# tenstack/batch-scheduler

Measured on AMD Instinct MI355X. Metric: pod x node fit evals/sec, higher is better.
Workload: dtype int64; 1 GPU; cfg3/tail: 10000 pods / 2000 groups / 5000 nodes, 5 int64 lanes (cpu, mem, eph, pods, gpu), seed 20260921; stages=prefilter+filter+tally+ready, parallelism=single GPU

## Files before the change

### batch-scheduler_amd/csrc/bs_fast.hpp

```cpp
#pragma once

#include "bs_kernels.hpp"
#include "bs_filter_t.hpp"

#ifdef BS_NT_TABLES
#define BS_TBL_STORE(p, v) __builtin_nontemporal_store((v), (p))
#else
#define BS_TBL_STORE(p, v) (*(p) = (v))
#endif
namespace bs {

template <bool INL = false>
__device__ __forceinline__ void arm_tally(const GroupsDev& gr, const BatchDev& b, const BatchParams& prm, uint32_t i, uint32_t nthreads);

__device__ __forceinline__ const uint8_t* range_glocal(const BatchDev& b) { return reinterpret_cast<const uint8_t*>(b.pod_ranges); }
__device__ __forceinline__ const uint32_t* range_start(const BatchDev& b, uint32_t G) { return b.pod_ranges + (G + 3u) / 4u; }
__device__ __forceinline__ const uint32_t* range_lfirst(const BatchDev& b, uint32_t G, uint32_t pod_blocks) { return range_start(b, G) + pod_blocks + 1u; }
__device__ __forceinline__ bool range_local_on(const BatchDev& b, const BatchParams& prm) {
  return b.pod_ranges && prm.do_tally && prm.do_ready && !prm.filter_deny;
}

#if BS_EMIT_MAIN
__global__ void k_pods_prep(unsigned long long* tables, uint32_t ntab, uint32_t* gstat, uint32_t ngstat, uint32_t* kcount, uint32_t* gcount, uint32_t G) {
  const uint32_t t = blockIdx.x * blockDim.x + threadIdx.x, nt = gridDim.x * blockDim.x;
  for (uint32_t i = t; i < ntab; i += nt) tables[i] = 0ull;
  for (uint32_t i = t; i < G; i += nt) gcount[i] = 0;
  for (uint32_t i = t; i < ngstat; i += nt) gstat[i] = BS_INF;
  if (t == 0 && kcount) *kcount = 0;
}
#endif

#if BS_EMIT_MAIN
__global__ void k_pod_pairs(PodsDev pods, uint32_t G, const uint32_t* rep, const uint32_t* id, uint32_t* pclass, unsigned long long* slots, uint32_t mask,
                            uint32_t hash_keep, uint32_t* gstat, uint32_t* ppair, unsigned long long* pair_next, const uint32_t* kcount, int32_t tag,
                            int32_t* hinfo, uint32_t* gcount) {
  const uint32_t i = blockIdx.x * blockDim.x + threadIdx.x;
  if (i == 0 && hinfo) {
    __hip_atomic_store(reinterpret_cast<unsigned long long*>(&hinfo[4]), ((unsigned long long)(uint32_t)tag << 32) | *kcount, __ATOMIC_RELAXED, __HIP_MEMORY_SCOPE_SYSTEM);
  }
  {
    const int32_t gq = i < pods.p ? pods.group[i] : -1;
    const bool in = gq >= 0 && (uint32_t)gq < G;
    wave_aggregated_add(gcount, in ? (uint32_t)gq : 0u, in);
  }
  if (i >= pods.p) return;
  const uint32_t c = id[rep[i]];
  if (pclass) pclass[i] = c;
  const int32_t gi = pods.group[i];
  if (gi < 0 || (uint32_t)gi >= G) { ppair[i] = BS_INF; return; }
  atomicMin(&gstat[gi], i);
  if (!(pods.flags[i] & BS_POD_LAST_PERMITTED)) {
    atomicMin(&gstat[(size_t)G + gi], i);
    if (pods.owner[i] != 0) atomicMin(&gstat[(size_t)2 * G + gi], i);
  }
  const uint64_t h = mix64(((uint64_t)(uint32_t)gi << 32) | c);
  bool winner;
// ... 447 lines not shown
      b.nodew[nodew_pair(stride, s, w) + 1] = ~holds;
    }
    if (blk == 0 && threadIdx.x == 0) {
#pragma unroll
      for (int j = 0; j < 4; ++j) b.nodew[nodew_ref_lane(stride, s, j)] = (uint64_t)ms.v[j];
      b.nodew[nodew_ref_flags(stride, s)] = ff;
    }
  }
}

template <int TS>
__global__ __launch_bounds__(kTblChunk) void k_fast_query_tables(PodsDev pods, GroupsDev gr, NodesDev nd, BatchDev b, BatchDev bt, BatchParams prm,
                                                                 const TableDesc* forced, uint32_t nchunks, uint32_t query_blocks) {
  BS_STAMP(1, 0);
  if (blockIdx.x < query_blocks) fast_query_thread<TS>(pods, gr, b, prm, blockIdx.x * kTblChunk + threadIdx.x, query_blocks * kTblChunk);
  else if (blockIdx.x < query_blocks + nchunks) tables_local_fast<TS>(nd, bt, prm, forced, blockIdx.x - query_blocks);
  else node_words_block<TS>(gr, nd, b, prm, blockIdx.x - query_blocks - nchunks);
  BS_STAMP(1, 7);
}

template <int NL>
__device__ __forceinline__ unsigned long long rows_cover(unsigned long long m, const int64_t (&a)[BS_MAX_LANES], const int64_t (&r)[BS_MAX_LANES]) {
  asm volatile("s_mov_b64 exec, %[m]\n\tv_cmpx_ge_i64 vcc, %[a0], %[r0]\n\tv_cmpx_ge_i64 vcc, %[a1], %[r1]\n\tv_cmpx_ge_i64 vcc, %[a2], %[r2]\n\t"
               "v_cmpx_ge_i64 vcc, %[a3], %[r3]\n\ts_mov_b64 %[m], exec\n\ts_mov_b64 exec, -1"
               : [m] "+s"(m)
               : [a0] "v"(a[0]), [r0] "v"(r[0]), [a1] "v"(a[1]), [r1] "v"(r[1]), [a2] "v"(a[2]), [r2] "v"(r[2]), [a3] "v"(a[3]), [r3] "v"(r[3])
               : "vcc");
#pragma unroll
  for (int j = 4; j < NL; ++j)
    asm volatile("s_mov_b64 exec, %[m]\n\tv_cmpx_ge_i64 vcc, %[a], %[r]\n\ts_mov_b64 %[m], exec\n\ts_mov_b64 exec, -1" : [m] "+s"(m) : [a] "v"(a[j]), [r] "v"(r[j]) : "vcc");
  return m;
}
#ifndef BS_SCAN_BALLOT
#define BS_SCAN_BALLOT 1
#endif
constexpr uint32_t kSpinBound = 1u << 18;
__device__ __forceinline__ void test_chaos_delay() {
#ifdef BS_TEST_CHAOS
  uint32_t h = (blockIdx.x + 1u) * 2654435761u ^ (uint32_t)wall_clock64() * 40503u;
  h ^= h >> 15; h *= 2246822519u; h ^= h >> 13;
  for (uint32_t s = 0; s < (h & 15u); ++s) __builtin_amdgcn_s_sleep(127);
#endif
}
constexpr uint32_t kStepSlotsMax = 256;
__device__ __forceinline__ bool step_wait(const uint32_t* word, uint32_t base, uint32_t need, int32_t* h_err) {
  uint32_t spins = 0;
  while ((uint32_t)(ld_agent(word) - base) < need) {
    __builtin_amdgcn_s_sleep(1);
    if (++spins > kSpinBound) { if (h_err) __hip_atomic_store(h_err, 1, __ATOMIC_RELAXED, __HIP_MEMORY_SCOPE_SYSTEM); return false; }
  }
  return true;
}
constexpr uint32_t kScanRecChunks = 64;
constexpr uint32_t kFeasRecGroups = 32;
#ifndef BS_GATHER_DIRECT
#define BS_GATHER_DIRECT 8
#endif
constexpr uint32_t kGatherDirectBlocks = BS_GATHER_DIRECT;
constexpr uint32_t kRecStride = 32;
constexpr uint32_t kTkSlots = 32, kTkTab = 48, kTkP1 = 64, kTkDone = 64 + 16 * 16, kTkWays = 16, kTkWords = 64 + 2 * 16 * 16;
__device__ __forceinline__ void spread_add(uint32_t* words, uint32_t who) {
  (void)__hip_atomic_fetch_add(&words[16u * (who % kTkWays)], 1u, __ATOMIC_RELAXED, __HIP_MEMORY_SCOPE_AGENT);
}
__device__ __forceinline__ bool spread_wait(const uint32_t* words, uint32_t base, uint32_t need, int32_t* h_err) {
  uint32_t spins = 0;
  for (;;) {
    uint32_t v = lane_id() < (int)kTkWays ? ld_agent(&words[16u * (uint32_t)lane_id()]) : 0u;
#pragma unroll
    for (int o = 1; o < (int)kTkWays; o <<= 1) v += (uint32_t)__shfl_xor((int)v, o);
    v = (uint32_t)__builtin_amdgcn_readfirstlane((int)v);
    if ((uint32_t)(v - base) >= need) return true;
    __builtin_amdgcn_s_sleep(4);
    if (++spins > kSpinBound) { if (h_err && lane_id() == 0) __hip_atomic_store(h_err, 1, __ATOMIC_RELAXED, __HIP_MEMORY_SCOPE_SYSTEM); return false; }
  }
}
template <int TS, bool REGS = false>
__device__ __forceinline__ void table_scan_block(const NodesDev& nd, const BatchDev& b, const BatchParams& prm, const TableDesc* forced, uint32_t chunk, uint32_t nchunks,
                                                 uint32_t share, uint32_t nshares, uint32_t pod_blocks, uint32_t tk_pods0, uint32_t tk_tab0, const GroupsDev& gr,
                                                 const int64_t* ckeys, const uint32_t* cpres, uint32_t kcap, bool direct = false, uint32_t forced_cls = 0) {
  __shared__ unsigned long long s_wtot[BS_MAX_LANES][4];
  __shared__ uint32_t s_kp[BS_MAX_SCALARS];
  __shared__ unsigned long long s_off[BS_MAX_LANES];
  __shared__ uint32_t s_kpg[BS_MAX_SCALARS];
  __shared__ int64_t s_req[kStepSlotsMax][BS_MAX_LANES];
  __shared__ uint32_t s_qf[kStepSlotsMax];
  __shared__ uint32_t s_first[kStepSlotsMax];
  BS_STAMP(2, 0);
  const Shape<TS> sh(prm.S);
  const uint32_t L = sh.L(), S = sh.S(), LP = prm.LP;
  const uint32_t k = chunk * kTblChunk + threadIdx.x;
  const bool in_range = REGS ? k < nd.n : k < nd.m;
  const uint32_t n = REGS ? (in_range ? k : 0u) : (in_range ? nd.kmap[k] : 0u);
  const TableDesc d = REGS ? TableDesc{forced_cls, 0.7f} : *forced;
  const uint32_t fw = nd.fit[(size_t)d.cls * nd.fit_words + (n >> 5)];
  const uint8_t fl = nd.flags[n];
  const bool valid = in_range && (!REGS || !(fl & BS_NODE_SKIP_MASK));
  const uint32_t ap = nd.apres[n], rp = nd.rpres[n];
  int64_t al[BS_MAX_LANES], rq[BS_MAX_LANES];
#pragma unroll
  for (uint32_t j = 0; j < BS_MAX_LANES; ++j) {
    if (j < L) {
      al[j] = nd.alloc[(size_t)j * nd.stride + n];
      rq[j] = nd.req[(size_t)j * nd.stride + n];
    }
  }
  const uint32_t K = prm.k_host ? prm.k_host : *b.kclass;
  const uint32_t per = (K + nshares - 1u) / nshares, s_lo = share * per, s_hi = min(K, s_lo + per);
// ... 147 lines not shown
    uint32_t stp = 0, qf = 0x80000000u;
    int32_t tab = -1;
    unsigned long long rv[BS_MAX_LANES];
    if (!REGS && t < s_hi) {
      stp = ld_agent(&b.qstamp_s[t]);
      tab = (int32_t)ld_agent(reinterpret_cast<const uint32_t*>(&b.qtab_s[t]));
      qf = ld_agent(&b.qflags_s[t]);
#pragma unroll
      for (uint32_t j = 0; j < BS_MAX_LANES; ++j) rv[j] = j < L ? ld_agent64(&b.qreq_s[(size_t)t * LP + j]) : 0ull;
    }
    if (w == 0) {
#pragma unroll
      for (uint32_t j = 0; j < BS_MAX_LANES; ++j) {
        if (j < L) {
          const unsigned long long incl_c = wave_incl_scan_add_u64(cv[j]);
          const unsigned long long mine = bcast64(incl_c - cv[j], (int)(chunk & 63u));
          if (ch == 0) s_off[j] = mine;
        }
      }
#pragma unroll
      for (uint32_t s2 = 0; s2 < BS_MAX_SCALARS; ++s2) {
        if (s2 < S) {
          const uint32_t mn = wave_min_u32(ckp[s2]);
          if (ch == 0) s_kpg[s2] = mn;
        }
      }
    }
    if (!REGS && t < s_hi) {
      if (stp != prm.stamp || tab != 0) qf = 0x80000000u;
      s_qf[threadIdx.x] = qf;
#pragma unroll
      for (uint32_t j = 0; j < BS_MAX_LANES; ++j)
        if (j < L) s_req[threadIdx.x][j] = (int64_t)rv[j];
    }
  }
  __syncthreads();
  if constexpr (REGS) {
    if (!s_ok) return;
  }
  int64_t fin[BS_MAX_LANES];
  uint32_t keyrow = 0;
#pragma unroll
  for (uint32_t j = 0; j < BS_MAX_LANES; ++j) {
    fin[j] = 0;
    if (j < L) fin[j] = (int64_t)(incl[j] + s_off[j]);
  }
#pragma unroll
  for (uint32_t s2 = 0; s2 < BS_MAX_SCALARS; ++s2)
    if (s2 < S && k >= s_kpg[s2]) keyrow |= 1u << s2;
  BS_STAMP(2, 3);
  const uint32_t nmine = s_hi > s_lo ? s_hi - s_lo : 0u;
  const uint32_t smask = S ? ((1u << S) - 1u) : 0u;
  const uint32_t row0 = chunk * kTblChunk + ((uint32_t)w << 6);
  for (uint32_t t0 = 0; t0 < nmine; t0 += 4u) {
    uint32_t qf[4];
    int64_t r[4][BS_MAX_LANES];
#pragma unroll
    for (uint32_t u = 0; u < 4; ++u) {
      const uint32_t t = min(t0 + u, nmine - 1u);
      qf[u] = t0 + u < nmine ? s_qf[t] : 0x80000000u;
#pragma unroll
      for (uint32_t j = 0; j < BS_MAX_LANES; ++j) r[u][j] = j < L ? s_req[t][j] : 0;
    }
#pragma unroll
    for (uint32_t u = 0; u < 4; ++u) {
      const uint32_t nab = ~(qf[u] >> 16) & smask;
      unsigned long long m = (qf[u] & 0x80000000u) ? 0ull : __ballot(valid && (nab & ~keyrow) == 0u);
      static_assert(TS >= 0 && TS <= 4, "k_fast_step_a is instantiated for 0..4 scalar lanes (run_fast: step_a_possible)");
#if BS_SCAN_BALLOT
#pragma unroll
      for (uint32_t j = 0; j < 4u + (uint32_t)TS; ++j) m &= __ballot(fin[j] >= r[u][j]);
#else
      m = rows_cover<4 + TS>(m, fin, r[u]);
#endif
      if (m && lane_id() == 0) atomicMin(&s_first[t0 + u], row0 + (uint32_t)(__ffsll((long long)m) - 1));
    }
  }
  __syncthreads();
  BS_STAMP(2, 4);
  if constexpr (REGS) {
    if (direct) {
      for (uint32_t t = threadIdx.x; t < nmine; t += kTblChunk)
        st_pub<true>(&b.scan_rec[(size_t)chunk * kStepSlotsMax + s_lo + t], ((unsigned long long)prm.seq_inv << 32) | s_first[t]);
    } else {
      for (uint32_t t = threadIdx.x; t < nmine; t += kTblChunk)
        if (s_first[t] != BS_INF) atomicMin(&b.first_row64[s_lo + t], ((unsigned long long)prm.seq_inv << 32) | s_first[t]);
    }
    BS_STAMP(2, 7);
    return;
  }
  for (uint32_t t = threadIdx.x; t < nmine; t += kTblChunk) {
    if (s_first[t] == BS_INF) continue;
    atomicMin(&b.first_row[s_lo + t], s_first[t]);
  }
  BS_STAMP(2, 7);
}

__device__ __forceinline__ void step_filter_split(uint32_t K, uint32_t W, uint32_t target_waves, uint32_t& tiles, uint32_t& bpw, uint32_t& nchunk) {
  tiles = (2u * K + 63u) / 64u;
  uint32_t nsplit = max(1u, target_waves / max(tiles, 1u));
  nsplit = min(nsplit, max((W + 1u) / 2u, 1u));
  bpw = max(2u, (((W + nsplit - 1u) / nsplit + 1u) / 2u) * 2u);
  nchunk = (W + bpw - 1u) / bpw;
  if ((nchunk + 3u) / 4u > kFeasRecGroups) {
    bpw = ((W + 4u * kFeasRecGroups - 1u) / (4u * kFeasRecGroups) + 1u) / 2u * 2u;
    nchunk = (W + bpw - 1u) / bpw;
  }
}
template <int TS>
__device__ __forceinline__ void step_filter_block(const GroupsDev& gr, const NodesDev& nd, const BatchDev& b, const BatchParams& prm, const int64_t* ckeys,
                                                  const uint32_t* cpres, uint32_t kcap, uint32_t target_waves, uint32_t ustride, uint32_t bx, uint32_t nblocks,
                                                  bool direct, uint32_t tk_slots0, uint32_t slot_producers) {
  __shared__ uint32_t s_cnt[4][64];
  BS_STAMP_AT(4, 0, bx);
  const Shape<TS> sh(prm.S);
  const uint32_t gate = prm.eph_gate, K = prm.k_host ? prm.k_host : (uint32_t)__builtin_amdgcn_readfirstlane((int)*b.kclass), U = 2u * K;
  const uint32_t W = (nd.n + 63u) / 64u;
  if (!U || !W) return;
  uint32_t tiles, bpw, nchunk;
  step_filter_split(K, W, target_waves, tiles, bpw, nchunk);
  const uint32_t groups = (nchunk + 3u) / 4u;
  const int32_t leader0 = b.leader_epoch[0];
  LeaderPre lp0{}, lp1{};
  const bool two = prm.sop_leader0 >= 0 && prm.sop_leader0 != leader0;
  if (gr.g) {
    leader_pre_load(gr, leader0, sh, lp0);
    if (two) leader_pre_load(gr, prm.sop_leader0, sh, lp1); else lp1 = lp0;
  }
  bool waited = false;
  for (uint32_t bi = bx; bi < tiles * groups; bi += nblocks) {
    const uint32_t tile = bi % tiles, group = bi / tiles, chunk = group * 4u + (uint32_t)wave_id();
    const uint32_t src = tile * 64u + (uint32_t)lane_id();
    const bool second = src >= K;
    const uint32_t c = src < U ? (second ? src - K : src) : 0u;
    uint32_t cnt = 0;
    if (chunk < nchunk) {
      Res raw;
#pragma unroll
      for (uint32_t j = 0; j < BS_MAX_LANES; ++j)
        if (j < sh.L()) raw.v[j] = ckeys[(size_t)j * kcap + c];
      raw.present = cpres[c];
      Res cur;
      res_zero(cur, sh);
      res_add(cur, raw, sh, gate);
      LeaderPre lp = lp0;
      if (second) lp = lp1;
      const bool on = src < U && (second ? prm.sop_leader0 >= 0 : leader0 >= 0) && lp.have_mr;
      int64_t R[4], M[4];
      const uint32_t ff = filter_slot_values(cur, lp, sh, gate, R, M);
      filter_item<2, 4, true, true>(nd, b, U, ustride, tile, chunk * bpw, min(W, chunk * bpw + bpw), 0u,
                                    on ? (ff | ((uint32_t)BS_FL_EVALUATED << 8)) : ((uint32_t)BS_FL_NOT_RUN << 8), R, M, &cnt);
    }
    s_cnt[wave_id()][lane_id()] = cnt;
    BS_STAMP_AT(4, 1, bx);
    if (direct && b.h_rows) asm volatile("s_waitcnt vmcnt(0)" ::: "memory");
    __syncthreads();
    BS_STAMP_AT(4, 2, bx);
    if (wave_id() == 0 && src < U) {
      const uint32_t sum = s_cnt[0][lane_id()] + s_cnt[1][lane_id()] + s_cnt[2][lane_id()] + s_cnt[3][lane_id()];
      if (direct) {
        st_pub<true>(&b.feas_rec[(size_t)group * (2u * kStepSlotsMax) + src], ((unsigned long long)prm.seq_inv << 32) | sum);
      } else {
        if (!waited) { (void)step_wait(&b.ticket[kTkSlots], tk_slots0, slot_producers, b.h_err); waited = true; }
        if (sum) atomicAdd(&b.fu_feas[src], sum);
      }
    }
    __syncthreads();
  }
  BS_STAMP_AT(4, 7, bx);
}

template <int TS>
__device__ __forceinline__ void class_slots_block(const GroupsDev& gr, const BatchDev& b, const BatchParams& prm, const int64_t* ckeys, const uint32_t* cpres,
                                                  uint32_t kcap, uint32_t blk, bool zero_feas) {
  const Shape<TS> sh(prm.S);
#ifdef BS_TEST_OLD_ZERO
  zero_feas = true;
#endif
  const uint32_t gate = prm.eph_gate, K = prm.k_host ? prm.k_host : *b.kclass;
  const uint32_t c = blk * kTblChunk + threadIdx.x;
  Res raw;
  const uint32_t cc = c < K ? c : 0u;
#pragma unroll
  for (uint32_t j = 0; j < BS_MAX_LANES; ++j)
    if (j < sh.L()) raw.v[j] = ckeys[(size_t)j * kcap + cc];
  raw.present = cpres[cc];
  const int32_t leader0 = b.leader_epoch[0];
  const uint8_t panic0 = b.panic_epoch[0];
  LeaderPre lp0{}, lp1{};
  const bool two = prm.run_filter && prm.sop_leader0 >= 0 && prm.sop_leader0 != leader0;
  if (gr.g) {
    leader_pre_load(gr, leader0, sh, lp0);
    if (two) leader_pre_load(gr, prm.sop_leader0, sh, lp1); else lp1 = lp0;
  }
  if (c < K) {
    Res cur;
    res_zero(cur, sh);
    res_add(cur, raw, sh, gate);
    if (leader0 >= 0 && !panic0) {
      Res q;
      const uint32_t qfw = class_scan_query(cur, lp0, sh, gate, q);
      int64_t* dst = b.qreq_s + (size_t)c * prm.LP;
#pragma unroll
      for (uint32_t j = 0; j < BS_MAX_LANES; ++j)
        if (j < prm.LP) st_pub<true>(&dst[j], j < sh.L() ? q.v[j] : (int64_t)INT64_MIN);
      st_pub<true>(&b.qflags_s[c], qfw);
      st_pub<true>(&b.qtab_s[c], (int32_t)0);
      st_pub<true>(&b.first_row[c], BS_INF);
      st_pub<true>(&b.qstamp_s[c], prm.stamp);
    }
    if (prm.run_filter) {
// ... 126 lines not shown
    __syncthreads();
  }
  const uint32_t dx = bx * 256u + threadIdx.x;
  const uint32_t i = p0 == BS_INF ? dx : p0 + threadIdx.x;
  const bool valid = i < pods.p && (p0 == BS_INF || i < p1);
  uint8_t code0 = 0, st0 = 0;
  int32_t gi0 = BS_POD_NOT_GROUPED;
  uint32_t qpos0 = 0, pclass0 = 0, pair0 = BS_INF;
  uint32_t lfirst = BS_INF;
  if (valid) { code0 = b.tcode[i]; st0 = b.stage[i]; gi0 = pods.group[i]; qpos0 = b.qpos[i]; pclass0 = b.pclass[i]; pair0 = b.ppair[i]; }
  if (INL && valid && range_local_on(b, prm)) lfirst = range_lfirst(b, gr.g, query_blocks)[i];
  const uint32_t K = prm.k_host ? prm.k_host : *b.kclass;
  const int32_t leader_now = b.leader_epoch[0];
  if (threadIdx.x < 64) {
    uint32_t found = BS_INF;
    for (uint32_t b0 = 0; b0 < query_blocks && found == BS_INF; b0 += 64u) {
      const uint32_t bk = b0 + threadIdx.x;
      uint32_t v = BS_INF;
      if (bk < query_blocks) {
        const unsigned long long w = INL ? ld_agent64(&b.first_reach64[bk]) : b.first_reach64[bk];
        if ((uint32_t)(w >> 32) == prm.seq_inv) v = (uint32_t)w;
      }
      const unsigned long long any = __ballot(v != BS_INF);
      if (any) found = (uint32_t)__shfl((int)v, __ffsll((long long)any) - 1);
    }
    if (threadIdx.x == 0) s_first_reach = found;
  }
  const bool owned = valid && (st0 & ST_OWNED);
  const bool walk = owned && (st0 & ST_ELIG);
  const bool grouped = valid && gi0 >= 0 && (uint32_t)gi0 < gr.g;
  uint32_t row_q = BS_INF, row_c = BS_INF, feas0 = 0, feas1 = 0;
  unsigned long long head = ~0ull, own_fq = ~0ull, own_next = ~0ull;
  if (walk) {
    head = b.pair_head[gi0];
    if (pair0 != BS_INF) { own_fq = INL ? ld_agent64(&b.pair_firstq[pair0]) : b.pair_firstq[pair0]; own_next = b.pair_next[pair0]; }
  }
  if constexpr (INL) {
    if (prm.do_tally && prm.do_ready) {
      uint32_t gwant = 0, gma = 0, gneed = 0;
      if (grouped) {
        gma = gr.matched[gi0];
        gneed = (uint32_t)(gr.min_member[gi0] - gr.status_scheduled[gi0]);
        gwant = lfirst != BS_INF ? kLocalTag | (lfirst - p0) : b.gcount[gi0];
      }
      s_gw[0][threadIdx.x] = gwant;
      s_gw[1][threadIdx.x] = gma;
      s_gw[2][threadIdx.x] = gneed;
    }
  }
  if (producers) {
    asm volatile("s_waitcnt vmcnt(0)" ::: "memory");
    if constexpr (INL) {
      const uint32_t tagw = prm.seq_inv, U = prm.run_filter ? 2u * K : 0u;
      uint32_t groups = 0;
      if (prm.run_filter) {
        uint32_t tiles, bpw, nchunk;
        step_filter_split(K, (nd.n + 63u) / 64u, aux, tiles, bpw, nchunk);
        groups = (nchunk + 3u) / 4u;
      }
      const unsigned long long none = ((unsigned long long)tagw << 32) | BS_INF, zero = (unsigned long long)tagw << 32;
      BS_STAMP(3, 4);
      if (query_blocks > kGatherDirectBlocks) {
        if (threadIdx.x < 64) (void)spread_wait(&b.ticket[kTkDone], tk_done, hint_blocks, b.h_err);
      } else
      for (uint32_t spins = 0;; ++spins) {
        uint32_t andt = tagw, ort = tagw, row = BS_INF, fs[2] = {0u, 0u};
        if (threadIdx.x < K) {
          const unsigned long long* rec = b.scan_rec + threadIdx.x;
          for (uint32_t c0 = 0; c0 < producers; c0 += 8u) {
            unsigned long long w[8];
#pragma unroll
            for (uint32_t u = 0; u < 8u; ++u) w[u] = c0 + u < producers ? ld_agent64(&rec[(size_t)(c0 + u) * kStepSlotsMax]) : none;
#pragma unroll
            for (uint32_t u = 0; u < 8u; ++u) { andt &= (uint32_t)(w[u] >> 32); ort |= (uint32_t)(w[u] >> 32); row = min(row, (uint32_t)w[u]); }
          }
        }
#pragma unroll
        for (uint32_t h = 0; h < 2u; ++h) {
          const uint32_t slot = threadIdx.x + 256u * h;
          if (slot < U) {
            const unsigned long long* rec = b.feas_rec + slot;
            for (uint32_t g0 = 0; g0 < groups; g0 += 8u) {
              unsigned long long w[8];
#pragma unroll
              for (uint32_t u = 0; u < 8u; ++u) w[u] = g0 + u < groups ? ld_agent64(&rec[(size_t)(g0 + u) * (2u * kStepSlotsMax)]) : zero;
#pragma unroll
              for (uint32_t u = 0; u < 8u; ++u) { andt &= (uint32_t)(w[u] >> 32); ort |= (uint32_t)(w[u] >> 32); fs[h] += (uint32_t)w[u]; }
            }
          }
        }
        const bool timed_out = spins > kSpinBound / 2u;
        if (__syncthreads_and((andt == tagw && ort == tagw) || timed_out)) {
          if (threadIdx.x < K) s_rowk[threadIdx.x] = row;
#pragma unroll
          for (uint32_t h = 0; h < 2u; ++h)
            if (threadIdx.x + 256u * h < U) s_feask[threadIdx.x + 256u * h] = fs[h];
          if (timed_out && threadIdx.x == 0 && b.h_err) __hip_atomic_store(b.h_err, 1, __ATOMIC_RELAXED, __HIP_MEMORY_SCOPE_SYSTEM);
          BS_COUNT(3, 5, spins + 1u);
          break;
        }
        __builtin_amdgcn_s_sleep(2);
      }
    } else if (threadIdx.x == 0) {
      uint32_t spins = 0;
      while (ld_agent(&b.ticket[1]) < producers) {
        __builtin_amdgcn_s_sleep(2);
        if (++spins > kSpinBound) { if (b.h_err) __hip_atomic_store(b.h_err, 1, __ATOMIC_RELAXED, __HIP_MEMORY_SCOPE_SYSTEM); break; }
      }
    }
  }
  __syncthreads();
  BS_STAMP(3, 1);
  const bool gathered = INL && query_blocks <= kGatherDirectBlocks;
  auto keyed_row = [&](uint32_t slot) -> uint32_t {
    if (gathered) return s_rowk[INL ? slot : 0u];
    const unsigned long long w = ld_agent64(&b.first_row64[slot]);
    return (uint32_t)(w >> 32) == prm.seq_inv ? (uint32_t)w : BS_INF;
  };
  if (owned && (st0 & ST_QUERY)) row_q = INL ? keyed_row(qpos0) : ld_agent(&b.first_row[qpos0]);
  if (walk) row_c = INL ? keyed_row(pclass0) : ld_agent(&b.first_row[pclass0]);
  if (valid && prm.run_filter && grouped) {
    if (gathered) { feas0 = s_feask[INL ? pclass0 : 0u]; feas1 = s_feask[INL ? pclass0 + K : 0u]; }
    else { feas0 = ld_agent(&b.fu_feas[pclass0]); feas1 = ld_agent(&b.fu_feas[pclass0 + K]); }
  }
  bool admit = false;
  if (valid) {
    uint8_t code = code0;
    const uint8_t st = st0;
    const int32_t gi = gi0;
    const uint32_t first_reach = min(s_first_reach, prm.first_reach_hint);
    uint32_t fk = BS_K_NOT_SCANNED;
    if (st & ST_OWNED) {
      bool denied = false;
// ... 328 lines not shown
```

### batch-scheduler_amd/csrc/bs_kernels.hpp

```cpp
#pragma once

#include "bs_common.hpp"
#include "bs_nodew_layout.hpp"

namespace bs {

struct NodesDev {
  uint32_t n, stride;
  const int64_t* alloc;
  const int64_t* req;
  const uint32_t* apres;
  const uint32_t* rpres;
  const uint8_t* flags;
  const uint32_t* fit;
  uint32_t fit_words, n_classes;
  const uint32_t* kmap;
  uint32_t m;
  const int64_t* left4;
  const int64_t* lglob;
};

struct GroupsDev {
  uint32_t g;
  const uint32_t* min_member;
// ... 1540 lines not shown
                 BS_OPT(f2, "v_cmpx_le_i64 vcc, %[R2], %[a2]\n\t") BS_OPT(f3, "v_cmpx_le_i64 vcc, %[R3], %[a3]\n\t")       \
                 "s_nop 3\n\t"                                                                                            \
                 "v_writelane_b32 %[vlo0], exec_lo, m0\n\t"                                                               \
                 "v_writelane_b32 %[vhi0], exec_hi, m0\n\t"                                                               \
                 "s_mov_b64 exec, %[ok1]\n\t"                                                                             \
                 BS_OPT(f0, "v_cmpx_le_i64 vcc, %[R0], %[b0]\n\t") BS_OPT(f1, "v_cmpx_le_i64 vcc, %[R1], %[b1]\n\t")       \
                 BS_OPT(f2, "v_cmpx_le_i64 vcc, %[R2], %[b2]\n\t") BS_OPT(f3, "v_cmpx_le_i64 vcc, %[R3], %[b3]\n\t")       \
                 "s_nop 3\n\t"                                                                                            \
                 "v_writelane_b32 %[vlo1], exec_lo, m0\n\t"                                                               \
                 "v_writelane_b32 %[vhi1], exec_hi, m0\n\t"                                                               \
                 "s_mov_b64 exec, -1"                                                                                     \
                 : [vlo0] "+v"(vlo0), [vhi0] "+v"(vhi0), [vlo1] "+v"(vlo1), [vhi1] "+v"(vhi1)                             \
                 : [pp] "s"(pp), [ok0] "s"(ok0), [ok1] "s"(ok1), [R0] "v"(R[0]), [R1] "v"(R[1]), [R2] "v"(R[2]),          \
                   [R3] "v"(R[3]), [a0] "v"(l0[0]), [a1] "v"(l0[1]), [a2] "v"(l0[2]), [a3] "v"(l0[3]), [b0] "v"(l1[0]),   \
                   [b1] "v"(l1[1]), [b2] "v"(l1[2]), [b3] "v"(l1[3])                                                      \
                 : "vcc");                                                                                                \
  }
BS_DEF_FILTER_POD2(1, 1, 0, 0, 0)
BS_DEF_FILTER_POD2(2, 0, 1, 0, 0)
BS_DEF_FILTER_POD2(3, 1, 1, 0, 0)
BS_DEF_FILTER_POD2(4, 0, 0, 1, 0)
BS_DEF_FILTER_POD2(5, 1, 0, 1, 0)
BS_DEF_FILTER_POD2(6, 0, 1, 1, 0)
BS_DEF_FILTER_POD2(7, 1, 1, 1, 0)
BS_DEF_FILTER_POD2(8, 0, 0, 0, 1)
BS_DEF_FILTER_POD2(9, 1, 0, 0, 1)
BS_DEF_FILTER_POD2(10, 0, 1, 0, 1)
BS_DEF_FILTER_POD2(11, 1, 1, 0, 1)
BS_DEF_FILTER_POD2(12, 0, 0, 1, 1)
BS_DEF_FILTER_POD2(13, 1, 0, 1, 1)
BS_DEF_FILTER_POD2(14, 0, 1, 1, 1)
BS_DEF_FILTER_POD2(15, 1, 1, 1, 1)

template <int MASK, int PU = 4>
__device__ __forceinline__ void filter_pod_loop(uint32_t np, const int64_t (*sR)[4], const unsigned long long (&okmask)[2],
                                                const int64_t (&l)[2][4], uint32_t (&vlo)[2], uint32_t (&vhi)[2]) {
  for (uint32_t pp = 0; pp < np; pp += PU) {
    int64_t R[PU][4];
#pragma unroll
    for (int u = 0; u < PU; ++u) {
      const uint32_t pu = min(pp + (uint32_t)u, np - 1);
#pragma unroll
      for (int j = 0; j < 4; ++j) R[u][j] = ((MASK >> j) & 1) ? sR[pu][j] : 0;
    }
#pragma unroll
    for (int u = 0; u < PU; ++u)
      filter_pod2<MASK>(min(pp + (uint32_t)u, np - 1), R[u], okmask[0], okmask[1], l[0], l[1], vlo[0], vhi[0], vlo[1], vhi[1]);
  }
}

template <int NB, int PU = 4, bool DB = true, bool REGS = false>
__device__ __forceinline__ void filter_item(const NodesDev& nd, const BatchDev& b, uint32_t U, uint32_t ustride, uint32_t ptile,
                                            uint32_t w0, uint32_t w1, uint32_t stamp = 0, uint32_t ff_in = 0, const int64_t* R_in = nullptr,
                                            const int64_t* M_in = nullptr, uint32_t* cnt_out = nullptr) {
  static_assert(NB == 2, "the inner statement handles two node blocks");
  typedef const __attribute__((address_space(4))) uint32_t* cflag_t;
  const int lane = lane_id();
  const uint32_t p0 = ptile * 64u;
  const uint32_t np = min(64u, U - p0);

  const bool mine = (uint32_t)lane < np;
  const uint32_t src = p0 + (uint32_t)lane;
  uint32_t myff = (uint32_t)BS_FL_NOT_RUN << 8;
  int64_t M[4] = {0, 0, 0, 0}, myR[4] = {0, 0, 0, 0};
  if constexpr (REGS) {
    if (mine) {
      myff = ff_in;
#pragma unroll
      for (int j = 0; j < 4; ++j) { myR[j] = R_in[j]; M[j] = M_in[j]; }
    }
  } else if (mine) {
    myff = b.uflags[src];
    const int64_t* rs = b.uparams + (size_t)src * 8;
#pragma unroll
    for (int j = 0; j < 4; ++j) { myR[j] = rs[j]; M[j] = rs[4 + j]; }
  }
  int64_t gl[8];
#pragma unroll
  for (int j = 0; j < 8; ++j) gl[j] = nd.lglob[j];
  int64_t l[NB][4], ln[NB][4];
  uint8_t nfl[NB], nfln[NB];
  auto load_blocks = [&](uint32_t w, int64_t (&dst)[NB][4], uint8_t (&fl)[NB]) {
#pragma unroll
    for (int nb = 0; nb < NB; ++nb) {
      const uint32_t n = (w + nb) * 64u + (uint32_t)lane;
      const bool nvalid = (w + nb) < w1 && n < nd.n;
      fl[nb] = 0xFF;
#pragma unroll
      for (int j = 0; j < 4; ++j) dst[nb][j] = INT64_MIN;
      if (nvalid) {
#pragma unroll
        for (int j = 0; j < 4; ++j) dst[nb][j] = nd.left4[(size_t)j * nd.stride + n];
        fl[nb] = nd.flags[n];
      }
    }
  };
  load_blocks(w0, l, nfl);
  if (!REGS && stamp) myff = (myff >> 16) == stamp ? (myff & 0xFFFFu) : ((uint32_t)BS_FL_NOT_RUN << 8);
  const uint32_t myfl = myff >> 8;
  const bool ev = myfl == BS_FL_EVALUATED;
  if (!ev) {
#pragma unroll
    for (int j = 0; j < 4; ++j) M[j] = 0;
  }
  __shared__ int64_t s_R[4][64][4];
  __builtin_amdgcn_wave_barrier();
  uint32_t lane_mask = 0;
  bool tile_allfail = false;
  {
#pragma unroll
    for (int j = 0; j < 4; ++j) s_R[wave_id()][lane][j] = myR[j];
    __builtin_amdgcn_wave_barrier();
// ... 349 lines not shown
```

### batch-scheduler_amd/csrc/bsched.hip

```cpp
#include <dlfcn.h>
#include <hip/hip_runtime.h>

#include <algorithm>
#include <cstdio>
#include <cstdlib>
#include <cstring>
#include <new>
#include <string>
#include <vector>

#ifndef BS_UNITY
#define BS_TU_MAIN
#endif
#include "bs_ctx.hpp"
#include "bs_fast.hpp"
#include "bs_epoch.hpp"
#include "bs_sort.hpp"
#include "bs_fit.hpp"
#include "bs_queue.hpp"
#include "bs_fdeny.hpp"
#include "bs_launch.hpp"
#ifdef BS_UNITY
#include "tu_fast.hip"
#include "tu_seq.hip"
// ... 1567 lines not shown
  return (uint64_t)ts.tv_sec * 1000000000ull + (uint64_t)ts.tv_nsec;
}
static bool step_a_possible(const bs_ctx* c, uint32_t stages, uint32_t k, uint32_t nchunks) {
  return c->step_a_on && !c->no_fuse_final && k > 0 && k <= kStepSlotsMax && nchunks <= 64 && c->M > 0 && c->P > 0 && !c->collect_stats &&
         c->cfg.enable_timing < 2 && c->S <= 4;
}
static int step_a_residency(bs_ctx* c, bool whole) {
  int& r = c->step_a_resident[whole ? 1 : 0];
  if (r < 0) r = step_a_residency_query(fast_launch(c), whole);
  return r;
}

static int run_fast(bs_ctx* c, uint32_t stages) {
  int rc;
  const uint32_t P = c->P, G = c->G, N = c->N;
  const uint32_t W = cdiv(N, 64);
  const bool run_filter = stages & BS_STAGE_FILTER;
  const bool commit = stages & BS_BATCH_COMMIT;
  NodesDev nd = nodes_dev(c);
  GroupsDev gr = groups_dev(c);
  PodsDev pd = pods_dev(c);
  BatchDev b = batch_dev(c);
  BatchParams prm = batch_params(c);
  prm.run_filter = run_filter;
  prm.use_classes = 1;
  prm.fuse_filter = run_filter ? 1u : 0u;
  prm.scan_slots_cap = c->scan_slots_cap;
  prm.filter_slots_cap = c->filter_slots_cap;
  prm.stamp = 1u + c->stamp_ctr;
  prm.seq_inv = ~c->key_seq;
  prm.commit = commit ? 1u : 0u;
  prm.do_tally = (stages & BS_STAGE_TALLY) ? 1u : 0u;
  prm.do_ready = (prm.do_tally && c->nranks == 1 && !c->reduce_external) ? 1u : 0u;
  if ((rc = setup_host_out(c, stages, run_filter, b, prm))) return rc;
  const uint32_t side_slot = (uint32_t)c->steady_table;
  const uint32_t nchunks = std::max<uint32_t>(1, cdiv(c->M, 256));
  BatchDev bt = b;
  bt.tables = b.tables + (size_t)side_slot * prm.mcap * prm.LP;
  bt.kp = b.kp + (size_t)side_slot * 16;
  bt.chunk_tot = b.chunk_tot + (size_t)side_slot * cdiv(c->Ncap, 256) * 16;
  bt.chunk_kp = b.chunk_kp + (size_t)side_slot * cdiv(c->Ncap, 256) * 16;
  bt.gmax = b.gmax + (size_t)side_slot * cdiv(c->Ncap, 64) * prm.LP;
  const TableDesc* forced = b.desc + side_slot;
  if (commit && G) HIPCHK(c, hipMemsetAsync(c->d_fast_reject.p, 0xFF, (size_t)G * 4, c->stream));

  if (c->kinfo_pending && ((volatile int32_t*)c->h_info.p)[5] == c->kinfo_tag && (rc = resolve_pods(c))) return rc;
  prm.k_host = c->kinfo_pending ? 0u : c->h_K;
  const uint64_t hp1 = c->host_probe ? host_ns() : 0;
  const bool k_known = !c->kinfo_pending;
  const uint32_t k_step = k_known ? prm.k_host : ((c->step_a_form >= 3u && c->dirs_ready) ? c->k_bound : 0u);
  if (step_a_possible(c, stages, k_step, nchunks) && (c->step_a_form == 1u || c->dirs_ready || (c->batch_since_pods && c->pairs_ready && c->rep_valid && c->have_groups))) {
    const uint32_t K = k_step;
    const uint32_t nshares = std::max<uint32_t>(1, std::min<uint32_t>(c->step_shares, cdiv(K, 8)));
    const uint32_t fblocks = run_filter ? cdiv(std::min<uint32_t>(c->filter_waves, cdiv(2 * K, 64) * std::max<uint32_t>(1, cdiv(W, 2))), 4) : 0u;
    uint32_t pb = 0;
    if (c->step_a_form >= 2u) {
      if (!c->dirs_ready && c->batch_since_pods && c->pairs_ready && c->rep_valid && c->have_groups && (rc = build_dirs(c))) return rc;
      if (c->dirs_ready) pb = cdiv(K, kTblChunk);
    }
    const uint32_t nch_nodes = std::max<uint32_t>(1, cdiv(N, 256));
    const uint32_t whole = (c->step_a_form >= 3u && pb && nch_nodes <= 64 && c->d_first_row64.p && c->d_scan_rec.p && c->d_feas_rec.p && c->d_chunk_rec.p) ? 1u : 0u;
    const uint32_t nchunks_s = whole ? nch_nodes : nchunks;
    const bool ranges = whole && c->ranges_valid && c->nranges && c->d_pod_ranges.p;
    const uint32_t qb = ranges ? c->nranges : cdiv(P, kTblChunk);
    if (ranges) b.pod_ranges = c->d_pod_ranges.as<uint32_t>();
    const uint32_t grid = qb + pb + nchunks_s * nshares + fblocks;
    if ((k_known || whole) && (int)grid <= step_a_residency(c, whole != 0)) {
      TIMED(c, BS_KERNEL_QUERY, {
        launch_fast_step_a(fast_launch(c), dim3(grid), pd, gr, nd, b, bt, prm, forced, nchunks_s, qb, nshares, fblocks, c->tk_pods, c->tk_tab, pb,
                           c->d_ckeys.as<int64_t>(), c->d_cpres.as<uint32_t>(), c->pair_cap, whole, c->tk_p1, c->tk_done, side_slot - c->C);
      });
      c->tk_pods += pb ? pb : qb;
      if (!whole) c->tk_tab += nchunks_s;
      if (whole) {
        c->tk_p1 += qb;
        if (qb > kGatherDirectBlocks) c->tk_done += nchunks_s * nshares + fblocks;
      } else {
        TIMED(c, BS_KERNEL_RESOLVE, hipLaunchKernelGGL(k_fast_final, dim3(cdiv(P, 256)), dim3(256), 0, c->stream, pd, gr, nd, b, prm, cdiv(P, kTblChunk)));
      }
      c->launches = whole ? 1 : 2;
      c->last_step_a = true;
      if (c->test_timeout_after && --c->test_timeout_after == 0 && c->h_info.p) {
        HIPCHK(c, hipStreamSynchronize(c->stream));
        ((volatile int32_t*)c->h_info.p)[12] = 1;
      }
      if (prm.filter_deny && (rc = launch_filter_deny(c, pd, gr, nd, b, prm, true))) return rc;
      if (commit) {
        if (prm.filter_deny && (rc = launch_filter_deny_marks(c, b, prm, b.fast_reject))) return rc;
        if (G) hipLaunchKernelGGL(k_fast_commit, dim3(cdiv(G, 256)), dim3(256), 0, c->stream, pd, b, const_cast<uint8_t*>(gr.flags),
                                  const_cast<uint64_t*>(gr.occupied), G, prm.filter_deny ? b.fd_flag : nullptr);
        LAUNCHCHK(c, BS_KERNEL_RESOLVE);
        int32_t last = -1;
        HIPCHK(c, hipMemcpyAsync(&last, b.pf_leader + (P - 1), 4, hipMemcpyDeviceToHost, c->stream));
        if (G) HIPCHK(c, hipMemcpyAsync(c->h_gflags.data(), gr.flags, G, hipMemcpyDeviceToHost, c->stream));
        HIPCHK(c, hipStreamSynchronize(c->stream));
        if (!fd_commit_gated(c) && !handover_commit_gated(c)) c->sop_leader0 = last;
        c->launches++;
      }
      return batch_collective(c, stages, gr, b);
    }
  }
  c->last_step_a = false;
  const uint32_t k_est = std::min<uint32_t>(P, c->kinfo_pending ? std::max<uint32_t>(2 * c->h_K, 1024) : std::max<uint32_t>(c->h_K, 1));
  const bool node_words = run_filter && cdiv(k_est, 64) > 16 && c->tp_filter >= 5u && !c->no_nodew && c->d_nodew.p;
  if (node_words) {
    b.nodew = bt.nodew = c->d_nodew.as<uint64_t>();
    b.nodew_stride = bt.nodew_stride = nodew_stride(N);
    b.tiles2_min = bt.tiles2_min = c->tp_tmin * std::max<uint32_t>(1u, c->nranks);
  }
  TIMED(c, BS_KERNEL_QUERY, {
    const uint32_t qb = cdiv(P, kTblChunk);
    const dim3 qg(qb + nchunks + (node_words ? nodew_blocks(N) : 0u)), blk(kTblChunk);
    lanes_narrow(c->S, [&](auto s) {
      hipLaunchKernelGGL(HIP_KERNEL_NAME(k_fast_query_tables<decltype(s)::value>), qg, blk, 0, c->stream, pd, gr, nd, b, bt, prm, forced, nchunks, qb);
    });
// ... 1218 lines not shown
```

Measured before the change: 3734 billion evals/s.

## Prune pod scan with wave-max bound and shrink filter tiles to live pods

```diff
diff --git a/batch-scheduler_amd/csrc/bs_fast.hpp b/batch-scheduler_amd/csrc/bs_fast.hpp
--- a/batch-scheduler_amd/csrc/bs_fast.hpp
+++ b/batch-scheduler_amd/csrc/bs_fast.hpp
@@ -2,6 +2,7 @@
 
 #include "bs_kernels.hpp"
 #include "bs_filter_t.hpp"
+#include "bs_filter_split.hpp"
 
 #ifdef BS_NT_TABLES
 #define BS_TBL_STORE(p, v) __builtin_nontemporal_store((v), (p))
@@ -555,7 +556,6 @@
   return true;
 }
 constexpr uint32_t kScanRecChunks = 64;
-constexpr uint32_t kFeasRecGroups = 32;
 #ifndef BS_GATHER_DIRECT
 #define BS_GATHER_DIRECT 8
 #endif
@@ -809,28 +809,45 @@
   const uint32_t nmine = s_hi > s_lo ? s_hi - s_lo : 0u;
   const uint32_t smask = S ? ((1u << S) - 1u) : 0u;
   const uint32_t row0 = chunk * kTblChunk + ((uint32_t)w << 6);
-  for (uint32_t t0 = 0; t0 < nmine; t0 += 4u) {
-    uint32_t qf[4];
-    int64_t r[4][BS_MAX_LANES];
-#pragma unroll
-    for (uint32_t u = 0; u < 4; ++u) {
-      const uint32_t t = min(t0 + u, nmine - 1u);
-      qf[u] = t0 + u < nmine ? s_qf[t] : 0x80000000u;
-#pragma unroll
-      for (uint32_t j = 0; j < BS_MAX_LANES; ++j) r[u][j] = j < L ? s_req[t][j] : 0;
-    }
-#pragma unroll
-    for (uint32_t u = 0; u < 4; ++u) {
-      const uint32_t nab = ~(qf[u] >> 16) & smask;
-      unsigned long long m = (qf[u] & 0x80000000u) ? 0ull : __ballot(valid && (nab & ~keyrow) == 0u);
-      static_assert(TS >= 0 && TS <= 4, "k_fast_step_a is instantiated for 0..4 scalar lanes (run_fast: step_a_possible)");
+  static_assert(TS >= 0 && TS <= 4, "k_fast_step_a is instantiated for 0..4 scalar lanes (run_fast: step_a_possible)");
+  int64_t wmax[4 + TS];
+#pragma unroll
+  for (uint32_t j = 0; j < 4u + (uint32_t)TS; ++j) wmax[j] = readlane63_i64(wave_max_i64_lane63(valid ? fin[j] : INT64_MIN));
+  for (uint32_t sb = 0; sb < nmine; sb += 64u) {
+    const uint32_t ts = sb + (uint32_t)lane_id();
+    bool cand = ts < nmine;
+    if (cand) {
+      cand = !(s_qf[ts] & 0x80000000u);
+#pragma unroll
+      for (uint32_t j = 0; j < 4u + (uint32_t)TS; ++j) cand = cand && wmax[j] >= s_req[ts][j];
+    }
+    unsigned long long todo = __ballot(cand);
+    auto fetch = [&](unsigned long long mk, uint32_t& t, uint32_t& qf, int64_t (&r)[BS_MAX_LANES]) {
+      t = sb + (mk ? (uint32_t)(__ffsll((long long)mk) - 1) : 0u);
+      qf = s_qf[t];
+#pragma unroll
+      for (uint32_t j = 0; j < BS_MAX_LANES; ++j) r[j] = j < 4u + (uint32_t)TS ? s_req[t][j] : 0;
+    };
+    uint32_t t = 0, qf = 0;
+    int64_t r[BS_MAX_LANES];
+    fetch(todo, t, qf, r);
+    while (todo) {
+      todo &= todo - 1ull;
+      uint32_t tn = 0, qfn = 0;
+      int64_t rn[BS_MAX_LANES];
+      fetch(todo, tn, qfn, rn);
+      const uint32_t nab = ~(qf >> 16) & smask;
+      unsigned long long m = __ballot(valid && (nab & ~keyrow) == 0u);
 #if BS_SCAN_BALLOT
 #pragma unroll
-      for (uint32_t j = 0; j < 4u + (uint32_t)TS; ++j) m &= __ballot(fin[j] >= r[u][j]);
+      for (uint32_t j = 0; j < 4u + (uint32_t)TS; ++j) m &= __ballot(fin[j] >= r[j]);
 #else
-      m = rows_cover<4 + TS>(m, fin, r[u]);
-#endif
-      if (m && lane_id() == 0) atomicMin(&s_first[t0 + u], row0 + (uint32_t)(__ffsll((long long)m) - 1));
+      m = rows_cover<4 + TS>(m, fin, r);
+#endif
+      if (m && lane_id() == 0) atomicMin(&s_first[t], row0 + (uint32_t)(__ffsll((long long)m) - 1));
+      t = tn; qf = qfn;
+#pragma unroll
+      for (uint32_t j = 0; j < BS_MAX_LANES; ++j) r[j] = rn[j];
     }
   }
   __syncthreads();
@@ -853,17 +870,6 @@
   BS_STAMP(2, 7);
 }
 
-__device__ __forceinline__ void step_filter_split(uint32_t K, uint32_t W, uint32_t target_waves, uint32_t& tiles, uint32_t& bpw, uint32_t& nchunk) {
-  tiles = (2u * K + 63u) / 64u;
-  uint32_t nsplit = max(1u, target_waves / max(tiles, 1u));
-  nsplit = min(nsplit, max((W + 1u) / 2u, 1u));
-  bpw = max(2u, (((W + nsplit - 1u) / nsplit + 1u) / 2u) * 2u);
-  nchunk = (W + bpw - 1u) / bpw;
-  if ((nchunk + 3u) / 4u > kFeasRecGroups) {
-    bpw = ((W + 4u * kFeasRecGroups - 1u) / (4u * kFeasRecGroups) + 1u) / 2u * 2u;
-    nchunk = (W + bpw - 1u) / bpw;
-  }
-}
 template <int TS>
 __device__ __forceinline__ void step_filter_block(const GroupsDev& gr, const NodesDev& nd, const BatchDev& b, const BatchParams& prm, const int64_t* ckeys,
                                                   const uint32_t* cpres, uint32_t kcap, uint32_t target_waves, uint32_t ustride, uint32_t bx, uint32_t nblocks,
@@ -874,9 +880,8 @@
   const uint32_t gate = prm.eph_gate, K = prm.k_host ? prm.k_host : (uint32_t)__builtin_amdgcn_readfirstlane((int)*b.kclass), U = 2u * K;
   const uint32_t W = (nd.n + 63u) / 64u;
   if (!U || !W) return;
-  uint32_t tiles, bpw, nchunk;
-  step_filter_split(K, W, target_waves, tiles, bpw, nchunk);
-  const uint32_t groups = (nchunk + 3u) / 4u;
+  const FilterSplit fs = step_filter_split(K, W, target_waves, prm.sop_leader0);
+  const uint32_t tiles = fs.tiles, bpw = fs.bpw, nchunk = fs.nchunk, groups = fs.groups;
   const int32_t leader0 = b.leader_epoch[0];
   LeaderPre lp0{}, lp1{};
   const bool two = prm.sop_leader0 >= 0 && prm.sop_leader0 != leader0;
@@ -887,9 +892,11 @@
   bool waited = false;
   for (uint32_t bi = bx; bi < tiles * groups; bi += nblocks) {
     const uint32_t tile = bi % tiles, group = bi / tiles, chunk = group * 4u + (uint32_t)wave_id();
-    const uint32_t src = tile * 64u + (uint32_t)lane_id();
+    const uint32_t base = tile * fs.tw, np = min(fs.tw, fs.ulive - base);
+    const uint32_t src = base + (uint32_t)lane_id();
+    const bool mine = (uint32_t)lane_id() < np;
     const bool second = src >= K;
-    const uint32_t c = src < U ? (second ? src - K : src) : 0u;
+    const uint32_t c = mine ? (second ? src - K : src) : 0u;
     uint32_t cnt = 0;
     if (chunk < nchunk) {
       Res raw;
@@ -902,18 +909,18 @@
       res_add(cur, raw, sh, gate);
       LeaderPre lp = lp0;
       if (second) lp = lp1;
-      const bool on = src < U && (second ? prm.sop_leader0 >= 0 : leader0 >= 0) && lp.have_mr;
+      const bool on = mine && (second ? prm.sop_leader0 >= 0 : leader0 >= 0) && lp.have_mr;
       int64_t R[4], M[4];
       const uint32_t ff = filter_slot_values(cur, lp, sh, gate, R, M);
       filter_item<2, 4, true, true>(nd, b, U, ustride, tile, chunk * bpw, min(W, chunk * bpw + bpw), 0u,
-                                    on ? (ff | ((uint32_t)BS_FL_EVALUATED << 8)) : ((uint32_t)BS_FL_NOT_RUN << 8), R, M, &cnt);
+                                    on ? (ff | ((uint32_t)BS_FL_EVALUATED << 8)) : ((uint32_t)BS_FL_NOT_RUN << 8), R, M, &cnt, base, np);
     }
     s_cnt[wave_id()][lane_id()] = cnt;
     BS_STAMP_AT(4, 1, bx);
     if (direct && b.h_rows) asm volatile("s_waitcnt vmcnt(0)" ::: "memory");
     __syncthreads();
     BS_STAMP_AT(4, 2, bx);
-    if (wave_id() == 0 && src < U) {
+    if (wave_id() == 0 && mine) {
       const uint32_t sum = s_cnt[0][lane_id()] + s_cnt[1][lane_id()] + s_cnt[2][lane_id()] + s_cnt[3][lane_id()];
       if (direct) {
         st_pub<true>(&b.feas_rec[(size_t)group * (2u * kStepSlotsMax) + src], ((unsigned long long)prm.seq_inv << 32) | sum);
@@ -1146,11 +1153,11 @@
     asm volatile("s_waitcnt vmcnt(0)" ::: "memory");
     if constexpr (INL) {
       const uint32_t tagw = prm.seq_inv, U = prm.run_filter ? 2u * K : 0u;
-      uint32_t groups = 0;
+      uint32_t groups = 0, ulive = 0;
       if (prm.run_filter) {
-        uint32_t tiles, bpw, nchunk;
-        step_filter_split(K, (nd.n + 63u) / 64u, aux, tiles, bpw, nchunk);
-        groups = (nchunk + 3u) / 4u;
+        const FilterSplit fs = step_filter_split(K, (nd.n + 63u) / 64u, aux, prm.sop_leader0);
+        groups = fs.groups;
+        ulive = fs.ulive;
       }
       const unsigned long long none = ((unsigned long long)tagw << 32) | BS_INF, zero = (unsigned long long)tagw << 32;
       BS_STAMP(3, 4);
@@ -1172,7 +1179,7 @@
 #pragma unroll
         for (uint32_t h = 0; h < 2u; ++h) {
           const uint32_t slot = threadIdx.x + 256u * h;
-          if (slot < U) {
+          if (slot < ulive) {
             const unsigned long long* rec = b.feas_rec + slot;
             for (uint32_t g0 = 0; g0 < groups; g0 += 8u) {
               unsigned long long w[8];
diff --git a/batch-scheduler_amd/csrc/bs_filter_split.hpp b/batch-scheduler_amd/csrc/bs_filter_split.hpp
--- /dev/null
+++ b/batch-scheduler_amd/csrc/bs_filter_split.hpp
@@ -0,0 +1,46 @@
+#pragma once
+#include <cstdint>
+
+#if defined(__HIPCC__) || defined(__CUDACC__)
+#define BS_SPLIT_HD __host__ __device__ __forceinline__
+#else
+#define BS_SPLIT_HD inline
+#endif
+
+constexpr uint32_t kFeasRecGroups = 32;
+
+struct FilterSplit {
+  uint32_t ulive;
+  uint32_t tw;
+  uint32_t tiles;
+  uint32_t bpw;
+  uint32_t nchunk;
+  uint32_t groups;
+};
+
+BS_SPLIT_HD FilterSplit step_filter_split(uint32_t K, uint32_t W, uint32_t target_waves, int32_t sop_leader0) {
+  FilterSplit s;
+  s.ulive = sop_leader0 < 0 ? K : 2u * K;
+  const uint32_t maxruns = (W + 1u) / 2u > 1u ? (W + 1u) / 2u : 1u;
+  s.tw = 64u;
+  while (s.tw > 16u && (uint64_t)((s.ulive + s.tw - 1u) / s.tw) * maxruns < target_waves) s.tw >>= 1;
+  s.tiles = (s.ulive + s.tw - 1u) / s.tw;
+  uint32_t nsplit = target_waves / (s.tiles ? s.tiles : 1u);
+  if (nsplit < 1u) nsplit = 1u;
+  if (nsplit > maxruns) nsplit = maxruns;
+  s.bpw = (((W + nsplit - 1u) / nsplit + 1u) / 2u) * 2u;
+  if (s.bpw < 2u) s.bpw = 2u;
+  s.nchunk = (W + s.bpw - 1u) / s.bpw;
+  if ((s.nchunk + 3u) / 4u > kFeasRecGroups) {
+    s.bpw = ((W + 4u * kFeasRecGroups - 1u) / (4u * kFeasRecGroups) + 1u) / 2u * 2u;
+    s.nchunk = (W + s.bpw - 1u) / s.bpw;
+  }
+  s.groups = (s.nchunk + 3u) / 4u;
+  return s;
+}
+
+BS_SPLIT_HD uint32_t step_filter_blocks(const FilterSplit& s, uint32_t target_waves) {
+  const uint64_t items = (uint64_t)s.tiles * s.nchunk;
+  const uint32_t waves = items < target_waves ? (uint32_t)items : target_waves;
+  return (waves + 3u) / 4u;
+}
diff --git a/batch-scheduler_amd/csrc/bs_kernels.hpp b/batch-scheduler_amd/csrc/bs_kernels.hpp
--- a/batch-scheduler_amd/csrc/bs_kernels.hpp
+++ b/batch-scheduler_amd/csrc/bs_kernels.hpp
@@ -1616,12 +1616,12 @@
 template <int NB, int PU = 4, bool DB = true, bool REGS = false>
 __device__ __forceinline__ void filter_item(const NodesDev& nd, const BatchDev& b, uint32_t U, uint32_t ustride, uint32_t ptile,
                                             uint32_t w0, uint32_t w1, uint32_t stamp = 0, uint32_t ff_in = 0, const int64_t* R_in = nullptr,
-                                            const int64_t* M_in = nullptr, uint32_t* cnt_out = nullptr) {
+                                            const int64_t* M_in = nullptr, uint32_t* cnt_out = nullptr, uint32_t base_in = 0, uint32_t np_in = 0) {
   static_assert(NB == 2, "the inner statement handles two node blocks");
   typedef const __attribute__((address_space(4))) uint32_t* cflag_t;
   const int lane = lane_id();
-  const uint32_t p0 = ptile * 64u;
-  const uint32_t np = min(64u, U - p0);
+  const uint32_t p0 = REGS ? base_in : ptile * 64u;
+  const uint32_t np = REGS ? np_in : min(64u, U - p0);
 
   const bool mine = (uint32_t)lane < np;
   const uint32_t src = p0 + (uint32_t)lane;
diff --git a/batch-scheduler_amd/csrc/bsched.hip b/batch-scheduler_amd/csrc/bsched.hip
--- a/batch-scheduler_amd/csrc/bsched.hip
+++ b/batch-scheduler_amd/csrc/bsched.hip
@@ -1643,7 +1643,7 @@
   if (step_a_possible(c, stages, k_step, nchunks) && (c->step_a_form == 1u || c->dirs_ready || (c->batch_since_pods && c->pairs_ready && c->rep_valid && c->have_groups))) {
     const uint32_t K = k_step;
     const uint32_t nshares = std::max<uint32_t>(1, std::min<uint32_t>(c->step_shares, cdiv(K, 8)));
-    const uint32_t fblocks = run_filter ? cdiv(std::min<uint32_t>(c->filter_waves, cdiv(2 * K, 64) * std::max<uint32_t>(1, cdiv(W, 2))), 4) : 0u;
+    uint32_t fblocks = run_filter ? cdiv(std::min<uint32_t>(c->filter_waves, cdiv(2 * K, 64) * std::max<uint32_t>(1, cdiv(W, 2))), 4) : 0u;
     uint32_t pb = 0;
     if (c->step_a_form >= 2u) {
       if (!c->dirs_ready && c->batch_since_pods && c->pairs_ready && c->rep_valid && c->have_groups && (rc = build_dirs(c))) return rc;
@@ -1652,6 +1652,7 @@
     const uint32_t nch_nodes = std::max<uint32_t>(1, cdiv(N, 256));
     const uint32_t whole = (c->step_a_form >= 3u && pb && nch_nodes <= 64 && c->d_first_row64.p && c->d_scan_rec.p && c->d_feas_rec.p && c->d_chunk_rec.p) ? 1u : 0u;
     const uint32_t nchunks_s = whole ? nch_nodes : nchunks;
+    if (whole && run_filter) fblocks = step_filter_blocks(step_filter_split(K, W, c->filter_waves, prm.sop_leader0), c->filter_waves);
     const bool ranges = whole && c->ranges_valid && c->nranges && c->d_pod_ranges.p;
     const uint32_t qb = ranges ? c->nranges : cdiv(P, kTblChunk);
     if (ranges) b.pod_ranges = c->d_pod_ranges.as<uint32_t>();
```

Result: no change. 3768 billion evals/s (median of 5 runs) (+0.9%).
